# apple/ml-4m

Measured on AMD Instinct MI355X. Metric: multimodal tokens/sec (4M-B train step, whole job), higher is better.
Workload: dtype bf16; 1 GPU; 4M-B mod7 (fm_base_12e_12d_swiglu_nobias, 360.8M params, 8 input / 7 target modalities) masked-modeling train step, 224^2 token grids, 128 input + 128 target tokens/sample, AdamW; model=fm_base_12e_12d_swiglu_nobias, per_gpu_batch=256, global_batch=256, seq_len=256, parallelism=dp1

## Files before the change

include/fourm_hip.h:

```cpp
#ifndef FOURM_HIP_H
#define FOURM_HIP_H
#include <stdint.h>

#ifdef __cplusplus
extern "C" {
#endif

#define FM_ABI_VERSION 11
int fm_abi_version(void);
const char* fm_last_error(void);

enum fm_epilogue {
    FM_EPI_BF16 = 0,
    FM_EPI_GELU = 1,
    FM_EPI_RESIDUAL = 2,
    FM_EPI_SWIGLU = 3,
    FM_EPI_F32 = 4,
    FM_EPI_TANH = 5,
    FM_EPI_SWIGLU_BWD = 6,
    FM_EPI_GELU_BWD = 7
};

typedef struct fm_gemm_group {
    const void* W;
// ... 147 lines not shown
} fm_embed_bwd_mod;
typedef struct fm_embed_bwd_desc {
    fm_embed_bwd_mod mods[FM_MAX_MODS];
    const void* dx;
    const void* slot_mod; const void* slot_src; const void* slot_pos;
    void* d_mask_token;
    void* d_reg_tokens;
    int32_t n_mods, batch, dim, Nt, lddx, is_decoder;
} fm_embed_bwd_desc;
int fm_embed_bwd(const fm_embed_bwd_desc* desc, void* stream);

int fm_dense_decoder_mask(const int32_t* cs, const int16_t* mod, void* out, int B, int M, int causal, int use_cs,
                          int use_sep, void* stream);

enum fm_loss_type { FM_LOSS_MOD = 0, FM_LOSS_TOKEN = 1 };
#define FM_SEG_ROWS 256
int fm_segment_rows(const int32_t* head_of_row, int R, int n_heads, int32_t* seg_start, int32_t* seg_count,
                    int32_t* perm, int32_t* row_to_padded, int32_t* tile_group, int Rp, void* stream);
int fm_gather_rows(const void* src, int ld_src, const int32_t* perm, void* dst, int ld_dst, int Rp, int D, void* stream);
int fm_cross_entropy(void* logits, int ldl, const int32_t* perm, const int32_t* tile_group, const int64_t* target_ids,
                     const int32_t* vocab, const int32_t* seg_start, const int32_t* seg_count, const void* grad_scale,
                     int loss_type, int n_heads, int Rp, int max_vocab, void* row_loss, void* row_lse, void* head_loss,
                     void* total_loss, int write_grad, void* stream);

int fm_swiglu_bwd(const void* da, int ldda, const void* gu, int ldgu, void* dgu, int lddgu, int R, int H, int Hp, void* stream);
int fm_gelu_bwd(const void* dh, int lddh, const void* pre, int ldp, void* dpre, int lddp, int R, int H, int Hp, void* stream);
typedef struct fm_shadow_desc {
    const void* src; void* dst;
    int32_t ld_src, ld_dst, rows, cols, transpose, tile_start;
    const void* col_scale;
    int32_t dst_f32, reserved;
} fm_shadow_desc;
int fm_shadow_refresh(const fm_shadow_desc* descs, int n_descs, int total_tiles, void* stream);
#define FM_FOLD_MAX_JOBS 48
typedef struct fm_fold_grad_job {
    const void* dWp; const void* W; const void* gamma; void* gW; void* ggamma;
    int32_t rows, cols, ld_dwp, reserved;
} fm_fold_grad_job;
int fm_fold_colscale_grad(const fm_fold_grad_job* jobs, int n_jobs, void* stream);

int fm_cast_pad(const void* src, int ld_src, void* dst, int ld_dst, int rows, int cols, void* stream);
int fm_transpose_cast_pad(const void* src, int ld_src, void* dst, int ld_dst, int dst_cols, int rows, int cols, void* stream);
int fm_colsum(const void* dy, int ldy, void* db, int R, int N, void* stream);
int fm_f32_to_bf16(const void* src, void* dst, int64_t n, void* stream);
int fm_bf16_to_f32_scaled(const void* src, void* dst, int64_t n, float scale, void* stream);
int fm_add_bf16_f32(const void* x, const void* delta, void* out, int64_t n, void* stream);
// ... 145 lines not shown
```

ml-4m_amd/csrc/loss.hip:

```cpp
#include "common.h"
#include "fourm_hip.h"

namespace {

constexpr int SEG_ALIGN = FM_SEG_ROWS;

__global__ __launch_bounds__(1024) void segment_rows_kernel(const int32_t* __restrict__ head_of_row, int R, int n_heads,
                                                            int32_t* __restrict__ seg_start, int32_t* __restrict__ seg_count,
                                                            int32_t* __restrict__ perm, int32_t* __restrict__ row_to_padded,
                                                            int32_t* __restrict__ tile_group, int Rp) {
    __shared__ int cnt[FM_MAX_MODS];
    __shared__ int wtot[16];
    const int g = blockIdx.x, tid = threadIdx.x, lane = tid & 63, wave = tid >> 6;
    if (tid < FM_MAX_MODS) cnt[tid] = 0;
    __syncthreads();
    for (int r = tid; r < R; r += 1024) {
        const int hh = head_of_row[r];
        if (hh >= 0 && hh <= g) atomicAdd(&cnt[hh], 1);
    }
    __syncthreads();
    int start = 0;
    for (int m = 0; m < g; ++m) start += (cnt[m] + SEG_ALIGN - 1) / SEG_ALIGN * SEG_ALIGN;
    const int mine = cnt[g];
    const int padded = (mine + SEG_ALIGN - 1) / SEG_ALIGN * SEG_ALIGN;
// ... 105 lines not shown
        return;
    }
    float w;
    if (loss_type == FM_LOSS_MOD) {
        w = 1.0f / ((float)seg_count[g] * (float)n_heads);
    } else {
        float tot = 0.f;
        for (int mm = 0; mm < n_heads; ++mm) tot += (float)seg_count[mm] * (float)vocab[mm];
        w = (float)V / tot;
    }
    w *= gscale ? gscale[0] : 1.0f;
    const float lse = row_lse[pr];
    const int tgt = (int)target_ids[src];
    for (int c = threadIdx.x * 8; c < Vp; c += 256 * 8) {
        const uint4 p = *(const uint4*)(row + c);
        const uint32_t wd[4] = {p.x, p.y, p.z, p.w};
        float o[8];
#pragma unroll
        for (int e = 0; e < 8; ++e) {
            const float x = bf2f((bf16_t)((e & 1) ? (wd[e >> 1] >> 16) : (wd[e >> 1] & 0xffff)));
            o[e] = (c + e < V) ? (__expf(x - lse) - ((c + e) == tgt ? 1.f : 0.f)) * w : 0.f;
        }
        *(uint4*)(row + c) = make_uint4(pack2bf(o[0], o[1]), pack2bf(o[2], o[3]), pack2bf(o[4], o[5]), pack2bf(o[6], o[7]));
    }
}

__global__ __launch_bounds__(256) void loss_finalize_kernel(const float* __restrict__ row_loss, const int32_t* __restrict__ seg_start,
                                                            const int32_t* __restrict__ seg_count, const int32_t* __restrict__ vocab,
                                                            int n_heads, int loss_type, float* __restrict__ head_loss, float* __restrict__ total) {
    __shared__ float red[4];
    __shared__ float hl[FM_MAX_MODS];
    const int lane = threadIdx.x & 63, wave = threadIdx.x >> 6;
    for (int g = 0; g < n_heads; ++g) {
        const int s0 = seg_start[g], n = seg_count[g];
        float s = 0.f;
        for (int i = threadIdx.x; i < n; i += 256) s += row_loss[s0 + i];
        s = wave_sum(s);
        if (lane == 0) red[wave] = s;
        __syncthreads();
        if (threadIdx.x == 0) hl[g] = n > 0 ? ((red[0] + red[1]) + (red[2] + red[3])) / (float)n : 0.f;
        __syncthreads();
    }
    if (threadIdx.x == 0) {
        float tot = 0.f, wsum = 0.f;
        for (int g = 0; g < n_heads; ++g) {
            head_loss[g] = hl[g];
// ... 91 lines not shown

extern "C" int fm_cross_entropy(void* logits, int ldl, const int32_t* perm, const int32_t* tile_group, const int64_t* target_ids,
                                const int32_t* vocab, const int32_t* seg_start, const int32_t* seg_count, const void* grad_scale,
                                int loss_type, int n_heads, int Rp, int max_vocab, void* row_loss, void* row_lse, void* head_loss,
                                void* total_loss, int write_grad, void* stream) {
    FM_CHECK_ARG(logits && perm && tile_group && target_ids && vocab && seg_start && seg_count && row_loss && row_lse && head_loss && total_loss,
                 "fm_cross_entropy: null pointer");
    FM_CHECK_ARG(loss_type == FM_LOSS_MOD || loss_type == FM_LOSS_TOKEN, "fm_cross_entropy: invalid loss type %d", loss_type);
    FM_CHECK_ARG(ldl % 8 == 0 && ldl >= (max_vocab + 63) / 64 * 64, "fm_cross_entropy: ldl=%d too small for vocab %d", ldl, max_vocab);
    FM_CHECK_ARG((((uintptr_t)logits) & 15) == 0, "fm_cross_entropy: logits must be 16-byte aligned");
    if (!write_grad) {
        hipLaunchKernelGGL(ce_fwd_kernel, dim3(Rp), dim3(256), 0, (hipStream_t)stream, (const bf16_t*)logits, ldl, perm, tile_group,
                           (const long long*)target_ids, vocab, (float*)row_loss, (float*)row_lse);
        hipLaunchKernelGGL(loss_finalize_kernel, dim3(1), dim3(256), 0, (hipStream_t)stream, (const float*)row_loss, seg_start, seg_count,
                           vocab, n_heads, loss_type, (float*)head_loss, (float*)total_loss);
    } else {
        hipLaunchKernelGGL(ce_bwd_kernel, dim3(Rp), dim3(256), 0, (hipStream_t)stream, (bf16_t*)logits, ldl, perm, tile_group,
                           (const long long*)target_ids, vocab, seg_count, (const float*)grad_scale, loss_type, n_heads, (const float*)row_lse);
    }
    FM_CHECK_LAUNCH("fm_cross_entropy");
    return 0;
}

extern "C" int fm_cross_entropy_f32(void* logits, int ldl, const int32_t* perm, const int32_t* tile_group, const int64_t* target_ids,
                                    const int32_t* vocab, const int32_t* seg_start, const int32_t* seg_count, const void* grad_scale,
                                    int loss_type, int n_heads, int Rp, int max_vocab, void* row_loss, void* row_lse, void* head_loss,
                                    void* total_loss, int write_grad, void* stream) {
    FM_CHECK_ARG(logits && perm && tile_group && target_ids && vocab && seg_start && seg_count && row_loss && row_lse && head_loss && total_loss,
                 "fm_cross_entropy_f32: null pointer");
    FM_CHECK_ARG(loss_type == FM_LOSS_MOD || loss_type == FM_LOSS_TOKEN, "fm_cross_entropy_f32: invalid loss type %d", loss_type);
    FM_CHECK_ARG(ldl >= max_vocab, "fm_cross_entropy_f32: ldl=%d too small for vocab %d", ldl, max_vocab);
    hipLaunchKernelGGL(ce_f32_kernel, dim3(Rp), dim3(256), 0, (hipStream_t)stream, (float*)logits, ldl, perm, tile_group,
                       (const long long*)target_ids, vocab, seg_count, (const float*)grad_scale, loss_type, n_heads, (float*)row_loss,
                       (float*)row_lse, write_grad, SEG_ALIGN);
    if (!write_grad)
        hipLaunchKernelGGL(loss_finalize_kernel, dim3(1), dim3(256), 0, (hipStream_t)stream, (const float*)row_loss, seg_start, seg_count,
                           vocab, n_heads, loss_type, (float*)head_loss, (float*)total_loss);
    FM_CHECK_LAUNCH("fm_cross_entropy_f32");
    return 0;
}
```

ml-4m_amd/fourm/hip/_lib.py:

```python
import ctypes as C
import os

FM_MAX_MODS = 24
_LIB_PATH = os.environ.get("FOURM_HIP_LIB") or os.path.join(os.path.dirname(os.path.dirname(os.path.abspath(__file__))), "_lib", "libfourm_hip.so")


class FourmHipUnavailable(ImportError):
    pass


def _load():
    if not os.path.exists(_LIB_PATH):
        raise FourmHipUnavailable(
            f"{_LIB_PATH} is missing - build the gfx950 kernels first: python ml-4m_amd/build_ext.py "
            "(the 4M hot path has no fallback implementation)")
    return C.CDLL(_LIB_PATH)


lib = _load()
lib.fm_last_error.restype = C.c_char_p
lib.fm_abi_version.restype = C.c_int
ABI_VERSION = 11
if lib.fm_abi_version() != ABI_VERSION:
    raise FourmHipUnavailable(f"libfourm_hip.so ABI {lib.fm_abi_version()} != expected {ABI_VERSION}; rebuild")
# ... 116 lines not shown
    fn.argtypes = list(argtypes)
    fn.restype = C.c_int
    return fn


P = C.POINTER
gemm_nt = _sig("fm_gemm_nt", P(GemmNTArgs), vp)
gemm_tn = _sig("fm_gemm_tn", P(GemmTNArgs), vp)
gemm_tn_multi = _sig("fm_gemm_tn_multi", P(GemmTNJob), C.c_int, vp)
layernorm_fwd = _sig("fm_layernorm_fwd", vp, i32, vp, vp, vp, i32, i32, vp, vp, vp, i32, i32, f32, vp)
layernorm_fwd_res = _sig("fm_layernorm_fwd_res", vp, i32, vp, i32, vp, i32, vp, vp, vp, i32, i32, vp, vp, vp, i32, i32, f32, vp)
layernorm_bwd = _sig("fm_layernorm_bwd", vp, i32, vp, vp, i32, vp, vp, vp, vp, vp, i32, vp, i32, vp, vp, i32, i32, vp)
layernorm_bwd_h = _sig("fm_layernorm_bwd_h", vp, i32, vp, i32, vp, i32, vp, vp, vp, vp, vp, i32, vp, i32, vp, i32, i32, vp)
attn_fwd = _sig("fm_attn_fwd", P(AttnArgs), vp)
attn_bwd = _sig("fm_attn_bwd", P(AttnArgs), vp)
attn_decode = _sig("fm_attn_decode", P(AttnDecodeArgs), vp)
ATTN_DECODE_MAX_NK = 8192
select_embed = _sig("fm_select_embed", P(SelectDesc), vp)
embed_bwd = _sig("fm_embed_bwd", P(EmbedBwdDesc), vp)
dense_decoder_mask = _sig("fm_dense_decoder_mask", vp, vp, vp, i32, i32, i32, i32, i32, vp)
segment_rows = _sig("fm_segment_rows", vp, i32, i32, vp, vp, vp, vp, vp, i32, vp)
gather_rows = _sig("fm_gather_rows", vp, i32, vp, vp, i32, i32, i32, vp)
cross_entropy = _sig("fm_cross_entropy", vp, i32, vp, vp, vp, vp, vp, vp, vp, i32, i32, i32, i32, vp, vp, vp, vp, i32, vp)
swiglu_bwd = _sig("fm_swiglu_bwd", vp, i32, vp, i32, vp, i32, i32, i32, i32, vp)
gelu_bwd = _sig("fm_gelu_bwd", vp, i32, vp, i32, vp, i32, i32, i32, i32, vp)
cast_pad = _sig("fm_cast_pad", vp, i32, vp, i32, i32, i32, vp)
transpose_cast_pad = _sig("fm_transpose_cast_pad", vp, i32, vp, i32, i32, i32, i32, vp)
colsum = _sig("fm_colsum", vp, i32, vp, i32, i32, vp)
shadow_refresh = _sig("fm_shadow_refresh", vp, i32, i32, vp)
fold_colscale_grad = _sig("fm_fold_colscale_grad", vp, i32, vp)
headnorm_fwd = _sig("fm_headnorm_fwd", vp, i32, vp, vp, vp, i32, vp, i32, i32, C.c_float, vp)
headnorm_bwd = _sig("fm_headnorm_bwd", vp, i32, vp, i32, vp, vp, vp, i32, vp, vp, i32, i32, vp)
f32_to_bf16 = _sig("fm_f32_to_bf16", vp, vp, i64, vp)
bf16_to_f32_scaled = _sig("fm_bf16_to_f32_scaled", vp, vp, i64, f32, vp)
add_bf16_f32 = _sig("fm_add_bf16_f32", vp, vp, vp, i64, vp)
lib.fm_set_reserved_cus.argtypes = [C.c_int]
lib.fm_get_reserved_cus.restype = C.c_int
lib.fm_get_reserved_cus.argtypes = []
adamw = _sig("fm_adamw", vp, vp, vp, vp, i64, f32, f32, f32, f32, f32, i64, vp, vp, vp, vp)
adamw_shadow = _sig("fm_adamw_shadow", vp, i32, i32, f32, f32, f32, f32, f32, i64, vp, vp, vp, vp)
sumsq = _sig("fm_sumsq", vp, i64, vp, vp)
clip_coef = _sig("fm_clip_coef", vp, f32, vp, vp, vp)
sample_tokens = _sig("fm_sample_tokens", vp, i32, i32, i32, i32, f32, i32, f32, vp, vp, vp, vp)
maskgit_commit = _sig("fm_maskgit_commit", vp, vp, vp, i32, i32, i32, vp, i32, i32, vp, vp, vp, vp)
gemm_f32 = _sig("fm_gemm_f32", P(GemmF32Args), vp)
attn_f32_fwd = _sig("fm_attn_f32_fwd", P(AttnArgs), vp)
# ... 50 lines not shown
unet_attention = _sig("fm_unet_attention", vp, i32, vp, i32, i32, i32, i32, i32, vp)
unet_im2col_f32 = _sig("fm_unet_im2col_f32", vp, i32, i32, vp, i32, i32, i32, i32, vp, i32, i32, i32, i32, i32, i32, i32, i32, vp)
groupnorm_nhwc_f32 = _sig("fm_groupnorm_nhwc_f32", vp, i32, vp, i32, vp, vp, vp, i32, i32, i32, i32, i32, f32, i32, vp)
unet_attention_f32 = _sig("fm_unet_attention_f32", vp, i32, vp, i32, i32, i32, i32, i32, vp)
add_f32 = _sig("fm_add_f32", vp, i32, vp, i32, vp, i32, i64, i32, vp)
silu_f32 = _sig("fm_silu_f32", vp, vp, i64, vp)
timestep_embedding_f32 = _sig("fm_timestep_embedding_f32", vp, vp, i32, i32, i32, f32, vp)
unet_col2im_f32 = _sig("fm_unet_col2im_f32", vp, i32, vp, i32, i32, i32, i32, i32, i32, i32, i32, i32, vp)
groupnorm_nhwc_bwd_f32 = _sig("fm_groupnorm_nhwc_bwd_f32", vp, i32, vp, i32, vp, i32, vp, vp, vp, i32, vp, vp, vp, i32, vp, i32, i32, i32, i32, f32, i32, vp)
unet_attention_bwd_f32 = _sig("fm_unet_attention_bwd_f32", vp, i32, vp, i32, vp, i32, vp, i32, i32, i32, i32, vp)
silu_bwd_f32 = _sig("fm_silu_bwd_f32", vp, vp, vp, i64, vp)
diffusion_x0 = _sig("fm_diffusion_x0", vp, vp, f32, f32, vp, i64, vp)
quantile_abs = _sig("fm_quantile_abs", vp, i32, i64, f32, vp, vp)
diffusion_step = _sig("fm_diffusion_step", vp, vp, f32, f32, vp, vp, vp, f32, f32, f32, f32, vp, vp, i32, i64, vp)
lora_apply = _sig("fm_lora_apply", vp, i32, vp, i64, i64, vp, i64, i64, vp, i32, f32, vp, i32, i32, i32, i32, i32, i32, vp)
lora_grad = _sig("fm_lora_grad", vp, i32, vp, vp, i64, i64, f32, i32, i32, i32, i32, i32, vp)
vit_patch_rows = _sig("fm_vit_patch_rows", vp, vp, i32, i32, i32, i32, i32, i32, i32, vp)
vit_emb_rows = _sig("fm_vit_emb_rows", vp, vp, vp, i32, i32, i32, i32, vp)
vit_colsum = _sig("fm_vit_colsum", vp, i32, vp, i32, i32, vp, i64, vp)
EXPORTS = ["fm_attn_decode", "fm_vit_patch_rows", "fm_vit_emb_rows", "fm_vit_colsum", "fm_lora_apply", "fm_lora_grad", "fm_vq_assign_wide", "fm_memcodes_assign", "fm_convnext_block", "fm_split3_bf16", "fm_unet_im2col", "fm_groupnorm_nhwc", "fm_add_bf16", "fm_silu_f32_to_bf16", "fm_timestep_embedding", "fm_unet_attention", "fm_diffusion_x0", "fm_quantile_abs",
           "fm_diffusion_step", "fm_unpack_image_u8", "fm_unpack_ids_u16", "fm_unpack_mask_bits", "fm_decoder_attention_from_target", "fm_guidance_combine", "fm_image_mask", "fm_token_budgets", "fm_span_mask", "fm_vq_code_stats", "fm_vq_ema_update", "fm_vq_code_bias", "fm_vq_assign_bias", "fm_vq_code_stats_raw", "fm_vq_ema_update_euclid", "fm_vq_unpatchify", "fm_vq_latent_grad", "fm_tanh_bwd_f32", "fm_embed_rows_f32", "fm_vq_patchify_ex", "fm_vq_cls_emb_bwd", "fm_vq_latent_grad_normalized", "fm_abi_version", "fm_last_error", "fm_gemm_nt", "fm_set_gemm_nt_config", "fm_get_gemm_nt_config", "fm_set_reserved_cus", "fm_get_reserved_cus", "fm_bf16_to_f32_scaled", "fm_add_bf16_f32", "fm_scale_rows_bf16", "fm_gemm_tn", "fm_gemm_tn_multi", "fm_set_gemm_tn_config", "fm_get_gemm_tn_config", "fm_set_tn_transpose_read",
           "fm_get_tn_transpose_read", "fm_layernorm_fwd", "fm_layernorm_fwd_res", "fm_layernorm_bwd", "fm_layernorm_bwd_h", "fm_headnorm_fwd", "fm_headnorm_bwd", "fm_attn_fwd", "fm_attn_bwd",
           "fm_set_attn_transpose_read", "fm_get_attn_transpose_read", "fm_select_embed", "fm_embed_bwd",
           "fm_dense_decoder_mask", "fm_segment_rows", "fm_gather_rows", "fm_cross_entropy", "fm_swiglu_bwd",
           "fm_gelu_bwd", "fm_cast_pad", "fm_transpose_cast_pad", "fm_shadow_refresh", "fm_fold_colscale_grad", "fm_colsum", "fm_f32_to_bf16", "fm_adamw", "fm_adamw_shadow",
           "fm_sumsq", "fm_clip_coef", "fm_vq_patchify", "fm_l2norm_rows", "fm_vq_assign",
           "fm_sample_tokens", "fm_maskgit_commit", "fm_gemm_f32", "fm_attn_f32_fwd", "fm_attn_f32_bwd", "fm_layernorm_bwd_f32", "fm_headnorm_f32_fwd", "fm_headnorm_f32_bwd",
           "fm_swiglu_bwd_f32", "fm_gelu_bwd_f32", "fm_colsum_f32", "fm_cross_entropy_f32", "fm_lab_set",
           "fm_unet_im2col_f32", "fm_groupnorm_nhwc_f32", "fm_unet_attention_f32", "fm_add_f32", "fm_silu_f32", "fm_timestep_embedding_f32",
           "fm_unet_col2im_f32", "fm_groupnorm_nhwc_bwd_f32", "fm_unet_attention_bwd_f32", "fm_silu_bwd_f32"]


def check(rc: int):
    if rc != 0:
        raise RuntimeError(f"libfourm_hip: {lib.fm_last_error().decode()} (rc={rc})")
```

ml-4m_amd/fourm/hip/engine.py:

```python
import math
import os
import random
import weakref
from typing import Dict, List, Optional

import torch
import torch.nn as nn

from . import _lib as L
from . import ops

_WEIGHT_EPOCH = 0
FUSE_ACT_BWD = os.environ.get("FOURM_FUSE_ACT_BWD", "0") == "1"
HEADS_DENSE = os.environ.get("FOURM_HEADS_DENSE", "1") == "1"
HEADS_DENSE_MAX = int(os.environ.get("FOURM_HEADS_DENSE_MAX", "8"))
DEFER_RESIDUAL = os.environ.get("FOURM_DEFER_RESIDUAL", "1") == "1"
HOIST_CTX = os.environ.get("FOURM_HOIST_CTX", "1") == "1"
LN_BWD_FROM_H = os.environ.get("FOURM_LN_BWD_FROM_H", "1") == "1"
DP_RESERVE_ALWAYS = os.environ.get("FOURM_DP_RESERVE_ALWAYS", "0") == "1"


def bump_weight_epoch():
    global _WEIGHT_EPOCH
    _WEIGHT_EPOCH += 1


def ru(x, m):
    return (x + m - 1) // m * m


def is_lora(lin) -> bool:
    return hasattr(lin, "lora_down")


def check_lora_targets(model):
    from fourm.models.lora_utils import MAX_LORA_WIDTH, LoRAWrapper
    ok = set()
    for blk in model.encoder:
        ok |= {id(blk.attn.qkv), id(blk.attn.proj)}
    for blk in getattr(model, "decoder", ()):
        ok |= {id(blk.self_attn.qkv), id(blk.self_attn.proj), id(blk.cross_attn.q), id(blk.cross_attn.kv), id(blk.cross_attn.proj)}
# ... 670 lines not shown
                st["dec_layers"].append(dict(ckpt_in=y))
                y = self.decoder_block_fwd(blk, y, ctx, B, Mt, N, smask, emask, None, f"dec{i % 2}", defer_out=i + 1 < len(m.decoder),
                                           out_name=f"dec{i}.y_out", ctx_hat=ctx_hat)
                st["dec_layers"][-1]["dp"] = self._last_dp
                continue
            sv = {} if save else None
            y = self.decoder_block_fwd(blk, y, ctx, B, Mt, N, smask, emask, sv, f"dec{i}" if save else f"dec{i % 2}",
                                       defer_out=i + 1 < len(m.decoder), ctx_hat=ctx_hat)
            if save:
                st["dec_layers"].append(sv)
        if save:
            st.update(top=sv_top, x_final=x, y_final=y, ctx=ctx, emask=emask, smask=smask, ctx_hat=ctx_hat, sv_hat=sv_hat)
        return y, st

    def heads_setup(self, dec, y_final, save):
        m = self.model
        heads = dec["heads"]
        nH = len(heads)
        B, Mt, D = dec["B"], dec["Nt"], self.D
        R = B * Mt
        Rp = ops.padded_rows(R, nH)
        ws, dev, i32 = self.ws, self.device, torch.int32
        hs = dict(n=nH, Rp=Rp, heads=heads)
        hs["seg_start"], hs["seg_count"] = ws.get("heads.seg_start", (nH,), i32), ws.get("heads.seg_count", (nH,), i32)
        hs["perm"], hs["r2p"] = ws.get("heads.perm", (Rp,), i32), ws.get("heads.r2p", (R,), i32)
        hs["tile_group"] = ws.get("heads.tile_group", (Rp // ops.SEG,), i32)
        ops.segment_rows(dec["head_of_row"].view(-1), nH, hs["seg_start"], hs["seg_count"], hs["perm"], hs["r2p"], hs["tile_group"])
        sv = {} if save else None
        yp = ws.get("heads.yp", (Rp, D), self.adt)
        with ops._prof("fills"):
            yp.zero_()
        self._ln(m.decoder_norm, y_final, yp, R, sv, "dn", "heads", row_map=hs["r2p"])
        vocabs = [m.decoder_embeddings[h].vocab_size for h in heads]
        hs["vocabs"], hs["maxV"] = vocabs, max(vocabs)
        ldl = ru(hs["maxV"], 64)
        w_fwd = [self.w(m.decoder_embeddings[h].to_logits.weight) for h in heads]
        w_bwd = [self.wt(m.decoder_embeddings[h].to_logits.weight) for h in heads] if save else None
        key = tuple(t.data_ptr() for t in w_fwd) + (tuple(t.data_ptr() for t in w_bwd) if save else ())
        cache = getattr(self, "_head_groups", None)
        if cache is None or cache[0] != key:
            fwd = ops.make_groups([dict(W=t, N=v, K=D, ldw=D) for t, v in zip(w_fwd, vocabs)], dev)
            if self.fp32:
                bwd = ops.make_groups([dict(W=m.decoder_embeddings[h].to_logits.weight, N=D, K=v, ldw=D, transposed=1)
                                       for h, v in zip(heads, vocabs)], dev) if save else None
            else:
                bwd = ops.make_groups([dict(W=t, N=D, K=ru(v, 64), ldw=ru(v, 64)) for t, v in zip(w_bwd, vocabs)], dev) if save else None
            vt = torch.tensor(vocabs, dtype=i32, device=dev)
            self._head_groups = cache = (key, fwd, bwd, vt)
        hs["g_fwd"], hs["g_bwd"], hs["vocab_t"] = cache[1], cache[2], cache[3]
        logits = ws.get("heads.logits", (Rp, ldl), self.adt)
        if HEADS_DENSE and not self.fp32 and nH <= HEADS_DENSE_MAX and ops.heads_dense_ok(w_fwd, vocabs, logits):
            ops.gemm_nt_heads(yp, w_fwd, vocabs, hs["seg_start"], hs["seg_count"], logits, D)
        else:
            ops.gemm_nt_grouped(yp, hs["g_fwd"], hs["tile_group"], logits, hs["maxV"], max_K=D)
        hs.update(yp=yp, logits=logits, sv=sv)
        hs["row_loss"] = ws.get("heads.row_loss", (Rp,), torch.float32)
        hs["row_lse"] = ws.get("heads.row_lse", (Rp,), torch.float32)
        hs["head_loss"] = ws.get("heads.head_loss", (nH,), torch.float32)
        hs["total"] = ws.get("heads.total", (1,), torch.float32)
        return hs

    def loss_forward(self, dec, hs, loss_type):
        lt = L.LOSS_MOD if loss_type in ("mod", "modality") else L.LOSS_TOKEN
        hs["loss_type"] = lt
        ops.cross_entropy(hs["logits"], hs["perm"], hs["tile_group"], dec["target_ids"].view(-1), hs["vocab_t"], hs["seg_start"],
                          hs["seg_count"], hs["n"], hs["maxV"], hs["row_loss"], hs["row_lse"], hs["head_loss"], hs["total"], loss_type=lt)
        return hs["total"], hs["head_loss"]

    def dec_order(self, mod_dict):
        names = [n for n in mod_dict if n in self.model.decoder_embeddings]
        return random.sample(names, len(names))

    def train_forward(self, mod_dict, n_enc, n_dec, loss_type, save=True):
        if loss_type not in ("mod", "modality", "token"):
            raise ValueError("Invalid loss type")
        self.prepare()
        if save:
            self._ensure_flat()
        enc_names = [n for n in mod_dict if n in self.model.encoder_embeddings]
        enc = self.select(mod_dict, n_enc, False, enc_names, "enc.")
        dec = self.select(mod_dict, n_dec, True, self.dec_order(mod_dict), "dec.")
        y, st = self.trunk_forward(enc, dec, save)
        hs = self.heads_setup(dec, y, save)
        total, head_loss = self.loss_forward(dec, hs, loss_type)
        if save:
            self._ctx = dict(enc=enc, dec=dec, st=st, hs=hs)
        return total, head_loss, hs["heads"], hs["seg_count"]

    def _g(self, p):
        return self.grad_view(p) if p.requires_grad else None

    def _dW(self, dy, x, lin, R64, n_cols=None, dy_cols=None):
        g = self._g(lin.weight)
        N = lin.weight.shape[0] if n_cols is None else n_cols
        if g is not None:
            if self._dw_jobs is not None:
                self._dw_jobs.append((dy, x, g.view(g.shape[0], -1), N, lin.weight[0].numel(), R64))
            else:
                ops.gemm_tn(dy, x, g.view(g.shape[0], -1), N=N, K=lin.weight[0].numel(), R=R64)
        if lin.bias is not None and lin.bias.requires_grad:
            ops.colsum(dy, self.grad_view(lin.bias), N, R=R64)

    def _flush_dW(self):
        jobs, self._dw_jobs = self._dw_jobs, None
        ops.gemm_tn_multi(jobs)

    def _ln_bwd(self, norm, dy, x, sv, key, g, g_bf, R, dres, dy_row_map=None):
# ... 158 lines not shown
            for i in range(d.n_mods):
                d2.mods[i].d_table = None
                d2.mods[i].d_proj_bias = None
            d2.d_reg_tokens = None
            d2.dx, d2.lddx = dx_extra.data_ptr(), dx_extra.stride(0)
            with ops._prof("embed_bwd"):
                L.check(L.embed_bwd(ops.C.byref(d2), ops._stream()))

    def train_backward(self, grad_scale: torch.Tensor):
        c = self._ctx
        if c is None:
            raise RuntimeError("train_backward without a preceding training forward")
        self._ctx, self._dw_jobs = None, None
        if self.reducer is not None:
            self.reducer.begin()
            if getattr(self.reducer, "reserved_cus", 0):
                L.lib.fm_set_reserved_cus(int(self.reducer.reserved_cus))
        m, ws = self.model, self.ws
        enc, dec, st, hs = c["enc"], c["dec"], c["st"], c["hs"]
        B, N, Mt, D = enc["B"], enc["Nt"], dec["Nt"], self.D
        bf, f32 = self.adt, torch.float32
        Rq, Rc = B * Mt, B * N
        Rqp, Rcp = st["y_final"].shape[0], st["x_final"].shape[0]
        ops.cross_entropy(hs["logits"], hs["perm"], hs["tile_group"], dec["target_ids"].view(-1), hs["vocab_t"], hs["seg_start"],
                          hs["seg_count"], hs["n"], hs["maxV"], hs["row_loss"], hs["row_lse"], hs["head_loss"], hs["total"],
                          loss_type=hs["loss_type"], grad_scale=grad_scale, write_grad=True)
        dyp = ws.get("bwd.dyp", (hs["Rp"], D), bf)
        ops.gemm_nt_grouped(hs["logits"], hs["g_bwd"], hs["tile_group"], dyp, D, max_K=ru(hs["maxV"], 64))
        heads = [m.decoder_embeddings[h] for h in hs["heads"]]
        if any(h.to_logits.weight.requires_grad for h in heads):
            outs = [self.grad_view(h.to_logits.weight) if h.to_logits.weight.requires_grad else None for h in heads]
            key = tuple(o.data_ptr() if o is not None else 0 for o in outs)
            cache = getattr(self, "_head_tn_groups", None)
            if cache is None or cache[0] != key:
                cache = self._head_tn_groups = (key, ops.make_groups(
                    [dict(out=o, N=(v if o is not None else 0)) for o, v in zip(outs, hs["vocabs"])], self.device))
            tn = cache[1]
            ops.gemm_tn_grouped(hs["logits"], hs["yp"], tn, hs["seg_start"], hs["seg_count"], hs["n"], hs["maxV"], hs["Rp"], D)
        g = ws.get("bwd.g_dec", (Rqp, D), f32)
        g_bf = ws.get("bwd.g_dec_bf", (Rqp, D), bf)
        self._ln_bwd(m.decoder_norm, dyp, st["y_final"], hs["sv"], "dn", g, g_bf, Rq, dres=None, dy_row_map=hs["r2p"])
        self._stage("heads")
        dctx = ws.get("bwd.dctx", (Rcp, D), f32)
        dctx_bf = ws.get("bwd.dctx_bf", (Rcp, D), bf)
        Ld = len(m.decoder)
        ctx_hat = st.get("ctx_hat")
        if ctx_hat is None:
            with ops._prof("fills"):
                dctx.zero_()
# ... 53 lines not shown
```

ml-4m_amd/fourm/hip/ops.py:

```python
import contextlib
import ctypes as C
import threading
from typing import Optional

import torch

from . import _lib as L

_PROFILER = None


def set_profiler(p):
    global _PROFILER
    _PROFILER = p


class _Null:
    def __enter__(self):
        return self

    def __exit__(self, *a):
        return False


# ... 348 lines not shown
    return ru(R, SEG) + SEG * (n_heads - 1)


@_timed("heads_misc")
def segment_rows(head_of_row, n_heads, seg_start, seg_count, perm, row_to_padded, tile_group):
    L.check(L.segment_rows(_p(head_of_row), head_of_row.numel(), n_heads, _p(seg_start), _p(seg_count), _p(perm),
                           _p(row_to_padded), _p(tile_group), perm.numel(), _stream()))


@_timed("heads_misc")
def gather_rows(src, perm, dst, D):
    L.check(L.gather_rows(_p(src), _ld(src), _p(perm), _p(dst), _ld(dst), perm.numel(), D, _stream()))


@_timed("cross_entropy")
def cross_entropy(logits, perm, tile_group, target_ids, vocab, seg_start, seg_count, n_heads, max_vocab, row_loss, row_lse, head_loss,
                  total_loss, *, loss_type=L.LOSS_MOD, grad_scale=None, write_grad=False):
    fn = L.cross_entropy_f32 if logits.dtype == torch.float32 else L.cross_entropy
    L.check(fn(_p(logits), _ld(logits), _p(perm), _p(tile_group), _p(target_ids), _p(vocab), _p(seg_start),
                            _p(seg_count), _p(grad_scale), loss_type, n_heads, perm.numel(), max_vocab, _p(row_loss), _p(row_lse),
                            _p(head_loss), _p(total_loss), 1 if write_grad else 0, _stream()))


@_timed("swiglu_bwd")
def swiglu_bwd(da, gu, dgu, H, Hp, R=None):
    if da.dtype == torch.float32:
        return L.check(L.swiglu_bwd_f32(_p(da), _ld(da), _p(gu), _ld(gu), _p(dgu), _ld(dgu), da.shape[0] if R is None else R, H, Hp, _stream()))
    L.check(L.swiglu_bwd(_p(da), _ld(da), _p(gu), _ld(gu), _p(dgu), _ld(dgu), da.shape[0] if R is None else R, H, Hp, _stream()))


@_timed("gelu_bwd")
def gelu_bwd(dh, pre, dpre, H, Hp, R=None):
    if dh.dtype == torch.float32:
        return L.check(L.gelu_bwd_f32(_p(dh), _ld(dh), _p(pre), _ld(pre), _p(dpre), _ld(dpre), dh.shape[0] if R is None else R, H, _stream()))
    L.check(L.gelu_bwd(_p(dh), _ld(dh), _p(pre), _ld(pre), _p(dpre), _ld(dpre), dh.shape[0] if R is None else R, H, Hp, _stream()))


def cast_pad(src, dst):
    s2 = src.reshape(src.shape[0], -1)
    L.check(L.cast_pad(_p(s2), s2.stride(0), _p(dst), _ld(dst), s2.shape[0], s2.shape[1], _stream()))
    return dst


def transpose_cast_pad(src, dst):
    s2 = src.reshape(src.shape[0], -1)
    L.check(L.transpose_cast_pad(_p(s2), s2.stride(0), _p(dst), _ld(dst), dst.shape[1], s2.shape[0], s2.shape[1], _stream()))
# ... 188 lines not shown
```

Measured before the change: 1.167 million tokens/s.

## Fuse training cross-entropy forward and gradient into one register-resident pass

In training, the cross-entropy forward now computes the log-sum-exp and writes d(logits) in place in a single kernel that keeps the whole row in registers. Before, the backward re-read the logits in a second kernel. The grad scale is predicted from the previous step, and a cheap rescale kernel in the backward fixes the gradients only when the actual scale differs. The full zeroing of the padded head-input buffer is also replaced by a kernel that zeroes only the padding rows. The cost is heavier register use for large vocabularies, and an epoch check is added to reject a backward after an intervening forward.

Result: no change. 1.164 million tokens/s (-0.2%).

```diff
diff --git a/include/fourm_hip.h b/include/fourm_hip.h
--- a/include/fourm_hip.h
+++ b/include/fourm_hip.h
@@ -193,6 +193,14 @@
                      const int32_t* vocab, const int32_t* seg_start, const int32_t* seg_count, const void* grad_scale,
                      int loss_type, int n_heads, int Rp, int max_vocab, void* row_loss, void* row_lse, void* head_loss,
                      void* total_loss, int write_grad, void* stream);
+#define FM_CE_TRAIN_MAX_VOCAB 32768
+int fm_cross_entropy_train(void* logits, int ldl, const int32_t* perm, const int32_t* tile_group, const int64_t* target_ids,
+                           const int32_t* vocab, const int32_t* seg_start, const int32_t* seg_count, const void* pred_scale,
+                           void* used_scale, int loss_type, int n_heads, int Rp, int max_vocab, void* row_loss, void* row_lse,
+                           void* head_loss, void* total_loss, void* stream);
+int fm_cross_entropy_rescale(void* dlogits, int ldl, const int32_t* perm, const int32_t* tile_group, const int32_t* vocab,
+                             const void* used_scale, const void* grad_scale, void* pred_scale, int Rp, int max_vocab, void* stream);
+int fm_zero_pad_rows(const int32_t* perm, void* dst, int64_t ld_bytes, int Rp, int row_bytes, void* stream);
 
 int fm_swiglu_bwd(const void* da, int ldda, const void* gu, int ldgu, void* dgu, int lddgu, int R, int H, int Hp, void* stream);
 int fm_gelu_bwd(const void* dh, int lddh, const void* pre, int ldp, void* dpre, int lddp, int R, int H, int Hp, void* stream);
diff --git a/ml-4m_amd/csrc/loss.hip b/ml-4m_amd/csrc/loss.hip
--- a/ml-4m_amd/csrc/loss.hip
+++ b/ml-4m_amd/csrc/loss.hip
@@ -151,6 +151,139 @@
             o[e] = (c + e < V) ? (__expf(x - lse) - ((c + e) == tgt ? 1.f : 0.f)) * w : 0.f;
         }
         *(uint4*)(row + c) = make_uint4(pack2bf(o[0], o[1]), pack2bf(o[2], o[3]), pack2bf(o[4], o[5]), pack2bf(o[6], o[7]));
+    }
+}
+
+template <int MAXC>
+__global__ __launch_bounds__(256) __attribute__((amdgpu_waves_per_eu(4))) void ce_train_kernel(bf16_t* __restrict__ logits, int ldl, const int32_t* __restrict__ perm,
+                                                       const int32_t* __restrict__ tile_group, const long long* __restrict__ target_ids,
+                                                       const int32_t* __restrict__ vocab, const int32_t* __restrict__ seg_count,
+                                                       const float* __restrict__ pred_scale, float* __restrict__ used_scale, int loss_type,
+                                                       int n_heads, float* __restrict__ row_loss, float* __restrict__ row_lse) {
+    constexpr int NCH = MAXC / 2048;
+    typedef __attribute__((ext_vector_type(4))) unsigned int u4_t;
+    __shared__ float red_m[4], red_s[4];
+    __shared__ float lse_sh;
+    const int pr = blockIdx.x;
+    float gs = pred_scale[0];
+    if (!(fabsf(gs) > 0.f && fabsf(gs) < INFINITY)) gs = 1.0f;
+    if (pr == 0 && threadIdx.x == 0) used_scale[0] = gs;
+    const int g = tile_group[pr / SEG_ALIGN];
+    if (g < 0) return;
+    const int V = vocab[g];
+    const int Vp = (V + 63) / 64 * 64;
+    bf16_t* row = logits + (size_t)pr * ldl;
+    const int src = perm[pr];
+    if (src < 0) {
+        if (threadIdx.x == 0) { row_loss[pr] = 0.f; row_lse[pr] = 0.f; }
+        for (int c = threadIdx.x; c < Vp / 8; c += 256) *(uint4*)(row + c * 8) = make_uint4(0u, 0u, 0u, 0u);
+        return;
+    }
+    uint4 buf[NCH];
+#pragma unroll
+    for (int i = 0; i < NCH; ++i) {
+        const int c = (i * 256 + threadIdx.x) * 8;
+        buf[i] = make_uint4(0u, 0u, 0u, 0u);
+        if (c < Vp) { const u4_t t = __builtin_nontemporal_load((const u4_t*)(row + c)); buf[i] = make_uint4(t[0], t[1], t[2], t[3]); }
+    }
+    float m = -INFINITY, ssum = 0.f;
+#pragma unroll
+    for (int i = 0; i < NCH; ++i) {
+        const int c = (i * 256 + threadIdx.x) * 8;
+        if (c < V) {
+            const uint32_t w[4] = {buf[i].x, buf[i].y, buf[i].z, buf[i].w};
+            float v[8];
+#pragma unroll
+            for (int e = 0; e < 4; ++e) { v[2 * e] = bf2f((bf16_t)(w[e] & 0xffff)); v[2 * e + 1] = bf2f((bf16_t)(w[e] >> 16)); }
+            if (c + 8 > V) {
+#pragma unroll
+                for (int e = 0; e < 8; ++e) v[e] = c + e < V ? v[e] : -INFINITY;
+            }
+            float cm = v[0];
+#pragma unroll
+            for (int e = 1; e < 8; ++e) cm = fmaxf(cm, v[e]);
+            const float mn = fmaxf(m, cm);
+            float add = 0.f;
+#pragma unroll
+            for (int e = 0; e < 8; ++e) add += __expf(v[e] - mn);
+            ssum = ssum * __expf(m - mn) + add;
+            m = mn;
+        }
+    }
+#pragma unroll
+    for (int o = 32; o > 0; o >>= 1) {
+        const float m2 = __shfl_xor(m, o, 64), s2 = __shfl_xor(ssum, o, 64);
+        if (m2 > -INFINITY || m > -INFINITY) online_merge(m, ssum, m2, s2);
+    }
+    const int lane = threadIdx.x & 63, wave = threadIdx.x >> 6;
+    if (lane == 0) { red_m[wave] = m; red_s[wave] = ssum; }
+    __syncthreads();
+    const int tgt = (int)target_ids[src];
+    if (threadIdx.x == 0) {
+        float M = red_m[0], S = red_s[0];
+        for (int w = 1; w < 4; ++w)
+            if (red_m[w] > -INFINITY) online_merge(M, S, red_m[w], red_s[w]);
+        const float l = M + __logf(S);
+        row_lse[pr] = l;
+        row_loss[pr] = l - bf2f(row[tgt]);
+        lse_sh = l;
+    }
+    __syncthreads();
+    const float lse = lse_sh;
+    float w;
+    if (loss_type == FM_LOSS_MOD) {
+        w = 1.0f / ((float)seg_count[g] * (float)n_heads);
+    } else {
+        float tot = 0.f;
+        for (int mm = 0; mm < n_heads; ++mm) tot += (float)seg_count[mm] * (float)vocab[mm];
+        w = (float)V / tot;
+    }
+    w *= gs;
+#pragma unroll
+    for (int i = 0; i < NCH; ++i) {
+        const int c = (i * 256 + threadIdx.x) * 8;
+        if (c < Vp) {
+            const uint32_t wd[4] = {buf[i].x, buf[i].y, buf[i].z, buf[i].w};
+            float o[8];
+#pragma unroll
+            for (int e = 0; e < 8; ++e) {
+                const float x = bf2f((bf16_t)((e & 1) ? (wd[e >> 1] >> 16) : (wd[e >> 1] & 0xffff)));
+                o[e] = (c + e < V) ? (__expf(x - lse) - ((c + e) == tgt ? 1.f : 0.f)) * w : 0.f;
+            }
+            *(uint4*)(row + c) = make_uint4(pack2bf(o[0], o[1]), pack2bf(o[2], o[3]), pack2bf(o[4], o[5]), pack2bf(o[6], o[7]));
+        }
+    }
+}
+
+__global__ __launch_bounds__(256) void ce_rescale_kernel(bf16_t* __restrict__ logits, int ldl, const int32_t* __restrict__ perm,
+                                                         const int32_t* __restrict__ tile_group, const int32_t* __restrict__ vocab,
+                                                         const float* __restrict__ used_scale, const float* __restrict__ grad_scale,
+                                                         float* __restrict__ pred_scale) {
+    const int pr = blockIdx.x;
+    const float used = used_scale[0], actual = grad_scale[0];
+    if (pr == 0 && threadIdx.x == 0) pred_scale[0] = actual;
+    if (used == actual) return;
+    const int g = tile_group[pr / SEG_ALIGN];
+    if (g < 0 || perm[pr] < 0) return;
+    const int Vp = (vocab[g] + 63) / 64 * 64;
+    const float ratio = actual / used;
+    bf16_t* row = logits + (size_t)pr * ldl;
+    for (int c = threadIdx.x * 8; c < Vp; c += 256 * 8) {
+        const uint4 p = *(const uint4*)(row + c);
+        const uint32_t wd[4] = {p.x, p.y, p.z, p.w};
+        uint32_t o[4];
+#pragma unroll
+        for (int e = 0; e < 4; ++e) o[e] = pack2bf(bf2f((bf16_t)(wd[e] & 0xffff)) * ratio, bf2f((bf16_t)(wd[e] >> 16)) * ratio);
+        *(uint4*)(row + c) = make_uint4(o[0], o[1], o[2], o[3]);
+    }
+}
+
+__global__ __launch_bounds__(256) void zero_pad_rows_kernel(const int32_t* __restrict__ perm, char* __restrict__ dst, size_t ld_bytes, int Rp,
+                                                            int row_bytes) {
+    const int lane = threadIdx.x & 63, wave = threadIdx.x >> 6;
+    for (int pr = blockIdx.x * 4 + wave; pr < Rp; pr += gridDim.x * 4) {
+        if (perm[pr] >= 0) continue;
+        for (int c = lane; c < row_bytes / 16; c += 64) *(uint4*)(dst + (size_t)pr * ld_bytes + (size_t)c * 16) = make_uint4(0u, 0u, 0u, 0u);
     }
 }
 
@@ -288,6 +421,57 @@
     return 0;
 }
 
+extern "C" int fm_cross_entropy_train(void* logits, int ldl, const int32_t* perm, const int32_t* tile_group, const int64_t* target_ids,
+                                      const int32_t* vocab, const int32_t* seg_start, const int32_t* seg_count, const void* pred_scale,
+                                      void* used_scale, int loss_type, int n_heads, int Rp, int max_vocab, void* row_loss, void* row_lse,
+                                      void* head_loss, void* total_loss, void* stream) {
+    FM_CHECK_ARG(logits && perm && tile_group && target_ids && vocab && seg_start && seg_count && pred_scale && used_scale && row_loss &&
+                 row_lse && head_loss && total_loss, "fm_cross_entropy_train: null pointer");
+    FM_CHECK_ARG(loss_type == FM_LOSS_MOD || loss_type == FM_LOSS_TOKEN, "fm_cross_entropy_train: invalid loss type %d", loss_type);
+    FM_CHECK_ARG(max_vocab > 0 && max_vocab <= FM_CE_TRAIN_MAX_VOCAB, "fm_cross_entropy_train: vocab %d above %d (use the two-pass kernels)",
+                 max_vocab, FM_CE_TRAIN_MAX_VOCAB);
+    FM_CHECK_ARG(ldl % 8 == 0 && ldl >= (max_vocab + 63) / 64 * 64, "fm_cross_entropy_train: ldl=%d too small for vocab %d", ldl, max_vocab);
+    FM_CHECK_ARG((((uintptr_t)logits) & 15) == 0, "fm_cross_entropy_train: logits must be 16-byte aligned");
+    FM_CHECK_ARG(pred_scale != used_scale, "fm_cross_entropy_train: pred_scale and used_scale must be distinct");
+    const int Vp = (max_vocab + 63) / 64 * 64;
+#define FM_CE_TRAIN(MAXC)                                                                                                                   \
+    hipLaunchKernelGGL(ce_train_kernel<MAXC>, dim3(Rp), dim3(256), 0, (hipStream_t)stream, (bf16_t*)logits, ldl, perm, tile_group,         \
+                       (const long long*)target_ids, vocab, seg_count, (const float*)pred_scale, (float*)used_scale, loss_type, n_heads,  \
+                       (float*)row_loss, (float*)row_lse)
+    if (Vp <= 4096) FM_CE_TRAIN(4096);
+    else if (Vp <= 8192) FM_CE_TRAIN(8192);
+    else if (Vp <= 16384) FM_CE_TRAIN(16384);
+    else FM_CE_TRAIN(32768);
+#undef FM_CE_TRAIN
+    hipLaunchKernelGGL(loss_finalize_kernel, dim3(1), dim3(256), 0, (hipStream_t)stream, (const float*)row_loss, seg_start, seg_count, vocab,
+                       n_heads, loss_type, (float*)head_loss, (float*)total_loss);
+    FM_CHECK_LAUNCH("fm_cross_entropy_train");
+    return 0;
+}
+
+extern "C" int fm_cross_entropy_rescale(void* dlogits, int ldl, const int32_t* perm, const int32_t* tile_group, const int32_t* vocab,
+                                        const void* used_scale, const void* grad_scale, void* pred_scale, int Rp, int max_vocab, void* stream) {
+    FM_CHECK_ARG(dlogits && perm && tile_group && vocab && used_scale && grad_scale && pred_scale, "fm_cross_entropy_rescale: null pointer");
+    FM_CHECK_ARG(ldl % 8 == 0 && ldl >= (max_vocab + 63) / 64 * 64, "fm_cross_entropy_rescale: ldl=%d too small for vocab %d", ldl, max_vocab);
+    FM_CHECK_ARG((((uintptr_t)dlogits) & 15) == 0, "fm_cross_entropy_rescale: d(logits) must be 16-byte aligned");
+    FM_CHECK_ARG(pred_scale != used_scale, "fm_cross_entropy_rescale: pred_scale and used_scale must be distinct");
+    hipLaunchKernelGGL(ce_rescale_kernel, dim3(Rp), dim3(256), 0, (hipStream_t)stream, (bf16_t*)dlogits, ldl, perm, tile_group, vocab,
+                       (const float*)used_scale, (const float*)grad_scale, (float*)pred_scale);
+    FM_CHECK_LAUNCH("fm_cross_entropy_rescale");
+    return 0;
+}
+
+extern "C" int fm_zero_pad_rows(const int32_t* perm, void* dst, int64_t ld_bytes, int Rp, int row_bytes, void* stream) {
+    FM_CHECK_ARG(perm && dst && Rp > 0, "fm_zero_pad_rows: bad argument");
+    FM_CHECK_ARG(row_bytes > 0 && row_bytes % 16 == 0 && ld_bytes % 16 == 0 && ld_bytes >= row_bytes && (((uintptr_t)dst) & 15) == 0,
+                 "fm_zero_pad_rows: rows must be 16-byte aligned multiples of 16 bytes");
+    int grid = (Rp + 3) / 4;
+    if (grid > 4096) grid = 4096;
+    hipLaunchKernelGGL(zero_pad_rows_kernel, dim3(grid), dim3(256), 0, (hipStream_t)stream, perm, (char*)dst, (size_t)ld_bytes, Rp, row_bytes);
+    FM_CHECK_LAUNCH("fm_zero_pad_rows");
+    return 0;
+}
+
 extern "C" int fm_cross_entropy_f32(void* logits, int ldl, const int32_t* perm, const int32_t* tile_group, const int64_t* target_ids,
                                     const int32_t* vocab, const int32_t* seg_start, const int32_t* seg_count, const void* grad_scale,
                                     int loss_type, int n_heads, int Rp, int max_vocab, void* row_loss, void* row_lse, void* head_loss,
diff --git a/ml-4m_amd/fourm/hip/_lib.py b/ml-4m_amd/fourm/hip/_lib.py
--- a/ml-4m_amd/fourm/hip/_lib.py
+++ b/ml-4m_amd/fourm/hip/_lib.py
@@ -162,6 +162,10 @@
 segment_rows = _sig("fm_segment_rows", vp, i32, i32, vp, vp, vp, vp, vp, i32, vp)
 gather_rows = _sig("fm_gather_rows", vp, i32, vp, vp, i32, i32, i32, vp)
 cross_entropy = _sig("fm_cross_entropy", vp, i32, vp, vp, vp, vp, vp, vp, vp, i32, i32, i32, i32, vp, vp, vp, vp, i32, vp)
+cross_entropy_train = _sig("fm_cross_entropy_train", vp, i32, vp, vp, vp, vp, vp, vp, vp, vp, i32, i32, i32, i32, vp, vp, vp, vp, vp)
+cross_entropy_rescale = _sig("fm_cross_entropy_rescale", vp, i32, vp, vp, vp, vp, vp, vp, i32, i32, vp)
+zero_pad_rows = _sig("fm_zero_pad_rows", vp, vp, i64, i32, i32, vp)
+CE_TRAIN_MAX_VOCAB = 32768
 swiglu_bwd = _sig("fm_swiglu_bwd", vp, i32, vp, i32, vp, i32, i32, i32, i32, vp)
 gelu_bwd = _sig("fm_gelu_bwd", vp, i32, vp, i32, vp, i32, i32, i32, i32, vp)
 cast_pad = _sig("fm_cast_pad", vp, i32, vp, i32, i32, i32, vp)
@@ -258,7 +262,7 @@
            "fm_diffusion_step", "fm_unpack_image_u8", "fm_unpack_ids_u16", "fm_unpack_mask_bits", "fm_decoder_attention_from_target", "fm_guidance_combine", "fm_image_mask", "fm_token_budgets", "fm_span_mask", "fm_vq_code_stats", "fm_vq_ema_update", "fm_vq_code_bias", "fm_vq_assign_bias", "fm_vq_code_stats_raw", "fm_vq_ema_update_euclid", "fm_vq_unpatchify", "fm_vq_latent_grad", "fm_tanh_bwd_f32", "fm_embed_rows_f32", "fm_vq_patchify_ex", "fm_vq_cls_emb_bwd", "fm_vq_latent_grad_normalized", "fm_abi_version", "fm_last_error", "fm_gemm_nt", "fm_set_gemm_nt_config", "fm_get_gemm_nt_config", "fm_set_reserved_cus", "fm_get_reserved_cus", "fm_bf16_to_f32_scaled", "fm_add_bf16_f32", "fm_scale_rows_bf16", "fm_gemm_tn", "fm_gemm_tn_multi", "fm_set_gemm_tn_config", "fm_get_gemm_tn_config", "fm_set_tn_transpose_read",
            "fm_get_tn_transpose_read", "fm_layernorm_fwd", "fm_layernorm_fwd_res", "fm_layernorm_bwd", "fm_layernorm_bwd_h", "fm_headnorm_fwd", "fm_headnorm_bwd", "fm_attn_fwd", "fm_attn_bwd",
            "fm_set_attn_transpose_read", "fm_get_attn_transpose_read", "fm_select_embed", "fm_embed_bwd",
-           "fm_dense_decoder_mask", "fm_segment_rows", "fm_gather_rows", "fm_cross_entropy", "fm_swiglu_bwd",
+           "fm_dense_decoder_mask", "fm_segment_rows", "fm_gather_rows", "fm_cross_entropy", "fm_cross_entropy_train", "fm_cross_entropy_rescale", "fm_zero_pad_rows", "fm_swiglu_bwd",
            "fm_gelu_bwd", "fm_cast_pad", "fm_transpose_cast_pad", "fm_shadow_refresh", "fm_fold_colscale_grad", "fm_colsum", "fm_f32_to_bf16", "fm_adamw", "fm_adamw_shadow",
            "fm_sumsq", "fm_clip_coef", "fm_vq_patchify", "fm_l2norm_rows", "fm_vq_assign",
            "fm_sample_tokens", "fm_maskgit_commit", "fm_gemm_f32", "fm_attn_f32_fwd", "fm_attn_f32_bwd", "fm_layernorm_bwd_f32", "fm_headnorm_f32_fwd", "fm_headnorm_f32_bwd",
diff --git a/ml-4m_amd/fourm/hip/engine.py b/ml-4m_amd/fourm/hip/engine.py
--- a/ml-4m_amd/fourm/hip/engine.py
+++ b/ml-4m_amd/fourm/hip/engine.py
@@ -17,6 +17,7 @@
 DEFER_RESIDUAL = os.environ.get("FOURM_DEFER_RESIDUAL", "1") == "1"
 HOIST_CTX = os.environ.get("FOURM_HOIST_CTX", "1") == "1"
 LN_BWD_FROM_H = os.environ.get("FOURM_LN_BWD_FROM_H", "1") == "1"
+CE_ONEPASS = os.environ.get("FOURM_CE_ONEPASS", "1") == "1"
 DP_RESERVE_ALWAYS = os.environ.get("FOURM_DP_RESERVE_ALWAYS", "0") == "1"
 
 
@@ -733,14 +734,14 @@
         Rp = ops.padded_rows(R, nH)
         ws, dev, i32 = self.ws, self.device, torch.int32
         hs = dict(n=nH, Rp=Rp, heads=heads)
+        self._heads_epoch = hs["epoch"] = getattr(self, "_heads_epoch", 0) + 1
         hs["seg_start"], hs["seg_count"] = ws.get("heads.seg_start", (nH,), i32), ws.get("heads.seg_count", (nH,), i32)
         hs["perm"], hs["r2p"] = ws.get("heads.perm", (Rp,), i32), ws.get("heads.r2p", (R,), i32)
         hs["tile_group"] = ws.get("heads.tile_group", (Rp // ops.SEG,), i32)
         ops.segment_rows(dec["head_of_row"].view(-1), nH, hs["seg_start"], hs["seg_count"], hs["perm"], hs["r2p"], hs["tile_group"])
         sv = {} if save else None
         yp = ws.get("heads.yp", (Rp, D), self.adt)
-        with ops._prof("fills"):
-            yp.zero_()
+        ops.zero_pad_rows(hs["perm"], yp)
         self._ln(m.decoder_norm, y_final, yp, R, sv, "dn", "heads", row_map=hs["r2p"])
         vocabs = [m.decoder_embeddings[h].vocab_size for h in heads]
         hs["vocabs"], hs["maxV"] = vocabs, max(vocabs)
@@ -771,9 +772,22 @@
         hs["total"] = ws.get("heads.total", (1,), torch.float32)
         return hs
 
-    def loss_forward(self, dec, hs, loss_type):
+    def _ce_scale(self):
+        t = getattr(self, "_ce_scale_buf", None)
+        if t is None or t.device != self.device:
+            t = self._ce_scale_buf = torch.ones(2, dtype=torch.float32, device=self.device)
+        return t[0:1], t[1:2]
+
+    def loss_forward(self, dec, hs, loss_type, train=False):
         lt = L.LOSS_MOD if loss_type in ("mod", "modality") else L.LOSS_TOKEN
         hs["loss_type"] = lt
+        hs["onepass"] = bool(train and CE_ONEPASS and not self.fp32 and hs["maxV"] <= ops.CE_TRAIN_MAX_VOCAB)
+        if hs["onepass"]:
+            pred, used = self._ce_scale()
+            ops.cross_entropy_train(hs["logits"], hs["perm"], hs["tile_group"], dec["target_ids"].view(-1), hs["vocab_t"], hs["seg_start"],
+                                    hs["seg_count"], hs["n"], hs["maxV"], hs["row_loss"], hs["row_lse"], hs["head_loss"], hs["total"],
+                                    pred, used, loss_type=lt)
+            return hs["total"], hs["head_loss"]
         ops.cross_entropy(hs["logits"], hs["perm"], hs["tile_group"], dec["target_ids"].view(-1), hs["vocab_t"], hs["seg_start"],
                           hs["seg_count"], hs["n"], hs["maxV"], hs["row_loss"], hs["row_lse"], hs["head_loss"], hs["total"], loss_type=lt)
         return hs["total"], hs["head_loss"]
@@ -793,7 +807,7 @@
         dec = self.select(mod_dict, n_dec, True, self.dec_order(mod_dict), "dec.")
         y, st = self.trunk_forward(enc, dec, save)
         hs = self.heads_setup(dec, y, save)
-        total, head_loss = self.loss_forward(dec, hs, loss_type)
+        total, head_loss = self.loss_forward(dec, hs, loss_type, train=save)
         if save:
             self._ctx = dict(enc=enc, dec=dec, st=st, hs=hs)
         return total, head_loss, hs["heads"], hs["seg_count"]
@@ -998,9 +1012,16 @@
         bf, f32 = self.adt, torch.float32
         Rq, Rc = B * Mt, B * N
         Rqp, Rcp = st["y_final"].shape[0], st["x_final"].shape[0]
-        ops.cross_entropy(hs["logits"], hs["perm"], hs["tile_group"], dec["target_ids"].view(-1), hs["vocab_t"], hs["seg_start"],
-                          hs["seg_count"], hs["n"], hs["maxV"], hs["row_loss"], hs["row_lse"], hs["head_loss"], hs["total"],
-                          loss_type=hs["loss_type"], grad_scale=grad_scale, write_grad=True)
+        if hs["onepass"]:
+            if hs["epoch"] != self._heads_epoch:
+                raise RuntimeError("train_backward: another forward has overwritten the d(logits) its training forward left in the heads' buffers "
+                                   "(run the backward first, or set FOURM_CE_ONEPASS=0)")
+            pred, used = self._ce_scale()
+            ops.cross_entropy_rescale(hs["logits"], hs["perm"], hs["tile_group"], hs["vocab_t"], hs["maxV"], used, grad_scale, pred)
+        else:
+            ops.cross_entropy(hs["logits"], hs["perm"], hs["tile_group"], dec["target_ids"].view(-1), hs["vocab_t"], hs["seg_start"],
+                              hs["seg_count"], hs["n"], hs["maxV"], hs["row_loss"], hs["row_lse"], hs["head_loss"], hs["total"],
+                              loss_type=hs["loss_type"], grad_scale=grad_scale, write_grad=True)
         dyp = ws.get("bwd.dyp", (hs["Rp"], D), bf)
         ops.gemm_nt_grouped(hs["logits"], hs["g_bwd"], hs["tile_group"], dyp, D, max_K=ru(hs["maxV"], 64))
         heads = [m.decoder_embeddings[h] for h in hs["heads"]]
diff --git a/ml-4m_amd/fourm/hip/ops.py b/ml-4m_amd/fourm/hip/ops.py
--- a/ml-4m_amd/fourm/hip/ops.py
+++ b/ml-4m_amd/fourm/hip/ops.py
@@ -394,6 +394,30 @@
                             _p(head_loss), _p(total_loss), 1 if write_grad else 0, _stream()))
 
 
+CE_TRAIN_MAX_VOCAB = L.CE_TRAIN_MAX_VOCAB
+
+
+@_timed("cross_entropy")
+def cross_entropy_train(logits, perm, tile_group, target_ids, vocab, seg_start, seg_count, n_heads, max_vocab, row_loss, row_lse, head_loss,
+                        total_loss, pred_scale, used_scale, *, loss_type=L.LOSS_MOD):
+    if logits.dtype != torch.bfloat16:
+        raise RuntimeError("cross_entropy_train: bf16 logits only (the fp32 mode uses the two-pass kernels)")
+    L.check(L.cross_entropy_train(_p(logits), _ld(logits), _p(perm), _p(tile_group), _p(target_ids), _p(vocab), _p(seg_start), _p(seg_count),
+                                  _p(pred_scale), _p(used_scale), loss_type, n_heads, perm.numel(), max_vocab, _p(row_loss), _p(row_lse),
+                                  _p(head_loss), _p(total_loss), _stream()))
+
+
+@_timed("cross_entropy")
+def cross_entropy_rescale(dlogits, perm, tile_group, vocab, max_vocab, used_scale, grad_scale, pred_scale):
+    L.check(L.cross_entropy_rescale(_p(dlogits), _ld(dlogits), _p(perm), _p(tile_group), _p(vocab), _p(used_scale), _p(grad_scale),
+                                    _p(pred_scale), perm.numel(), max_vocab, _stream()))
+
+
+@_timed("fills")
+def zero_pad_rows(perm, dst):
+    L.check(L.zero_pad_rows(_p(perm), _p(dst), _ld(dst) * dst.element_size(), perm.numel(), dst.shape[1] * dst.element_size(), _stream()))
+
+
 @_timed("swiglu_bwd")
 def swiglu_bwd(da, gu, dgu, H, Hp, R=None):
     if da.dtype == torch.float32:
```
